# mmbajo/PROBA-V

Hardware: AMD Instinct MI355X
Metric: LR-patches/sec fwd+bwd (WDSR-B r12 t9, 16x16, bs128) (higher is better)
Workload: dtype f32 (products as 3 scaled-fp16-piece MFMA products, f32 accumulate)

## Files before the change

proba-v_amd/csrc/kernels_cw4.hip:

```cpp
#include "kernels_x6.h"
#include "x6_device.h"
#include <cstdlib>
#include <algorithm>

namespace probav {
#ifdef CW4_DIAG
namespace diag {
#endif

struct Cw4Args {
    ConvGeom g;
    int Wp, Wt, nsplit, SR, nstrips, nslot;
    unsigned mTo, mNvr, mTi, mNslot;
};

namespace {
__device__ __forceinline__ int qdiv(int v, int d, unsigned m) { return (int)__umulhi((unsigned)v, m) + (d == 1 ? v : 0); }
unsigned qmagic(int d) { return d <= 1 ? 0u : (unsigned)((0x100000000ull + (unsigned)d - 1) / (unsigned)d); }
typedef float f32x4u __attribute__((ext_vector_type(4), aligned(4)));
typedef unsigned u32x4b __attribute__((ext_vector_type(4)));
constexpr int CW4_PSE = 151;
constexpr int CW4_PS = 16 * CW4_PSE;
constexpr int CW4_ROW = 8 * CW4_PS;
constexpr unsigned CW4_OOB = 0x40000000u;
}

#ifdef CW4_STAMP
__device__ unsigned long long g_cw4_stamps[1024 * 8];
#endif

#define CW4_SBAR() __builtin_amdgcn_sched_barrier(0)
#ifdef CW4_STAMP
#define CW4_ST(k) do { unsigned long long t_; asm volatile("s_memtime %0\n\ts_waitcnt lgkmcnt(0)" : "=s"(t_) :: "memory"); st_acc[k] += t_ - st_prev; st_prev = t_; } while (0)
#ifdef CW4_STAMP_ROUNDS
#define CW4_STR(k) CW4_ST(k)
#else
#define CW4_STR(k) do { } while (0)
#endif
#else
#define CW4_STR(k) do { } while (0)
#define CW4_ST(k) do { } while (0)
#endif

template <int CIN, int COUT, int TP, bool RELU, bool SKIP, bool BIAS>
__global__ __launch_bounds__(256, 1) void conv3_w4_kernel(Cw4Args a, const float* __restrict__ x, const uint4* __restrict__ wfrag, const float* __restrict__ bias,
                                                         const float* __restrict__ skip, float* __restrict__ y, Amax am)
{
    extern __shared__ __attribute__((aligned(16))) unsigned char lds[];
    constexpr int NST = CIN == 25 ? 5 : 6, KB = 9 * NST, G = 3 * KB;
    constexpr int NW1R = CIN == 25 ? 12 : 8;
    constexpr int NCH = CIN == 25 ? 3 : 4;
    constexpr int PS = CW4_PS, ROW = CW4_ROW;
    constexpr int PD = 2;
    constexpr int TO = TP - 2;
    const ConvGeom& g = a.g;
    const int tid = threadIdx.x, lane = tid & 63, half = lane >> 5, col = lane & 31;
    const int wave = __builtin_amdgcn_readfirstlane(tid >> 6);
    const int per = a.nstrips * a.nsplit;
    const int n = blockIdx.x / per, srem = blockIdx.x - n * per;
    const int strip = srem / a.nsplit, sp = srem - strip * a.nsplit;
    const int ws0 = sp * a.Wt, hb = strip * a.SR;
    const int SRr = g.Ho - hb < a.SR ? g.Ho - hb : a.SR;
    const int nvr = a.Wt * g.To, NV = SRr * nvr, NTL = (NV + 31) >> 5, nround = (NTL + 3) >> 2;
    const int NS = a.nslot;
    float omax = 0.f;
#ifdef CW4_STAMP
    unsigned long long st_t0 = __builtin_amdgcn_s_memtime(), st_r0 = __builtin_amdgcn_s_memrealtime();
    unsigned long long st_prev = st_t0, st_acc[8] = {0, 0, 0, 0, 0, 0, 0, 0};
#endif

    const int lw0 = a.nsplit == 1 ? g.pw : 0, Wl = a.nsplit == 1 ? g.Wi : a.Wt + 2;
    const int nvs = Wl * g.Ti, items = nvs * NCH;
    const int ea = h3_exp(am.x[n]);
    const float sa = pow2i(ea);
    int s_srcb[2], s_offb[2];
    float s_sc[2];
    int s3_o[3], s3_offb = 0;
    float s3_sc[3] = {0.f, 0.f, 0.f};
    {
        auto locate = [&](int lv, int& lw, int& t, int& iwc, int& colok) {
            const int lwr = qdiv(lv, g.Ti, a.mTi);
            t = lv - lwr * g.Ti; lw = lw0 + lwr;
            const int iw = ws0 + lw - g.pw;
            colok = (iw >= 0 ? 1 : 0) & (iw < g.Wi ? 1 : 0);
            iwc = iw < 0 ? 0 : (iw < g.Wi ? iw : g.Wi - 1);
        };
#pragma unroll
        for (int k = 0; k < 2; ++k) {
            const int it = tid + 256 * k;
            const int ic = it < items ? it : items - 1;
            const int lv = CIN == 25 ? (int)(((unsigned)ic * 43691u) >> 17) : ic >> 2;
            const int cc = ic - lv * NCH;
            int lw, t, iwc, colok;
            locate(lv, lw, t, iwc, colok);
            s_srcb[k] = ((iwc * g.Ti + t) * CIN + 8 * cc) * 4;
            s_offb[k] = (lw * TO + t) * 16 + cc * PS;
            s_sc[k] = colok ? sa : 0.f;
        }
        if constexpr (CIN == 25) {
            const int lv = tid < nvs ? tid : nvs - 1;
            int lw, t, iwc, colok;
            locate(lv, lw, t, iwc, colok);
            const int base = ((iwc * g.Ti + t) * CIN + 24) * 4;
            s3_offb = (lw * TO + t) * 16 + 3 * PS;
            const int ok3[3] = {colok && t - 1 >= 0, colok, colok && t + 1 < g.Ti};
#pragma unroll
            for (int j = 0; j < 3; ++j) { s3_o[j] = base + (ok3[j] ? (j - 1) * CIN * 4 : 0); s3_sc[j] = ok3[j] ? sa : 0.f; }
        }
    }
    const long xsample = (long)g.Hi * g.Wi * g.Ti * CIN;
    const __amdgpu_buffer_rsrc_t xrs = __builtin_amdgcn_make_buffer_rsrc(const_cast<float*>(x + (long)n * xsample), 0, (unsigned)xsample * 4u, 0x00020000);
    const int xrowb = g.Wi * g.Ti * CIN * 4;
    struct Staged { u32x4b v[2][2]; unsigned g3[3]; };
    auto row_of = [&](int q, int& rowoff, float& rokf) {
        const int ih = hb - g.ph + q;
        const bool rok = ih >= 0 && ih < g.Hi;
        rowoff = (rok ? ih : 0) * xrowb;
        rokf = rok ? 1.f : 0.f;
    };
    auto stage_load_items = [&](int rowoff, Staged& sv) {
#pragma unroll
        for (int k = 0; k < 2; ++k) {
            sv.v[k][0] = __builtin_amdgcn_raw_buffer_load_b128(xrs, s_srcb[k], rowoff, 0);
            sv.v[k][1] = __builtin_amdgcn_raw_buffer_load_b128(xrs, s_srcb[k] + 16, rowoff, 0);
        }
    };
    auto stage_load_g3 = [&](int rowoff, Staged& sv) {
#ifdef CW4_ABL_NOG3
        sv.g3[0] = sv.g3[1] = sv.g3[2] = 0u; return;
#endif
        if constexpr (CIN == 25) {
#pragma unroll
            for (int j = 0; j < 3; ++j) sv.g3[j] = __builtin_amdgcn_raw_buffer_load_b32(xrs, s3_o[j], rowoff, 0);
        }
    };
    auto slot_of = [&](int q) -> int { return (q - qdiv(q, NS, a.mNslot) * NS) * ROW; };
    struct Cut { float sc[2], sg[3]; f32x2 t[4]; unsigned h0[4], h1[4]; float u[3]; };
    constexpr int ROW_MOPS = CIN == 25 ? 52 : 41;
    auto stage_mop = [&](int m, int slot, float rokf, Staged& sv, Cut& c, bool reload, int rel) {
        if (m < 5) {
            if (m < 2) c.sc[m] = s_sc[m] * rokf;
            else if (CIN == 25) c.sg[m - 2] = s3_sc[m - 2] * rokf;
            return;
        }
        m -= 5;
        if (m < 36) {
            const int k = m / 18, i = m % 18;
            if (i < 16) {
                const int p = i >> 2, op = i & 3;
                if (op == 0) {
                    const u32x4b q = sv.v[k][p >> 1];
                    const f32x2 v = {__uint_as_float(q[2 * (p & 1)]), __uint_as_float(q[2 * (p & 1) + 1])};
                    c.t[p] = v * (f32x2){c.sc[k], c.sc[k]};
                    if (p == 3 && reload) {
                        sv.v[k][0] = __builtin_amdgcn_raw_buffer_load_b128(xrs, s_srcb[k], rel, 0);
                        sv.v[k][1] = __builtin_amdgcn_raw_buffer_load_b128(xrs, s_srcb[k] + 16, rel, 0);
                    }
                } else if (op == 1) {
                    c.h0[p] = __builtin_bit_cast(unsigned, __builtin_convertvector(c.t[p], f16x2));
                } else if (op == 2) {
                    asm("v_fma_mixlo_f16 %0, %1, -1.0, %2 op_sel:[0,0,0] op_sel_hi:[1,0,0]" : "=v"(c.h1[p]) : "v"(c.h0[p]), "v"(c.t[p][0]));
                } else {
                    asm("v_fma_mixhi_f16 %0, %1, -1.0, %2 op_sel:[1,0,0] op_sel_hi:[1,0,0]" : "+v"(c.h1[p]) : "v"(c.h0[p]), "v"(c.t[p][1]));
                }
            } else {
#ifdef CW4_ABL_NOWRITE
                asm volatile("" :: "v"(c.h0[0]), "v"(c.h0[1]), "v"(c.h0[2]), "v"(c.h0[3]), "v"(c.h1[0]), "v"(c.h1[1]), "v"(c.h1[2]), "v"(c.h1[3]));
                return;
#endif
                unsigned char* ent = lds + slot + s_offb[k];
                if (i == 16) *reinterpret_cast<uint4*>(ent) = make_uint4(c.h0[0], c.h0[1], c.h0[2], c.h0[3]);
                else *reinterpret_cast<uint4*>(ent + 4 * PS) = make_uint4(c.h1[0], c.h1[1], c.h1[2], c.h1[3]);
            }
            return;
        }
        if constexpr (CIN == 25) {
            m -= 36;
            if (m < 3) { c.u[m] = __uint_as_float(sv.g3[m]) * c.sg[m]; if (m == 2 && reload) stage_load_g3(rel, sv); }
            else if (m == 3) c.h0[0] = __builtin_bit_cast(unsigned, __builtin_convertvector((f32x2){c.u[0], c.u[1]}, f16x2));
            else if (m == 4) c.h0[1] = __builtin_bit_cast(unsigned, __builtin_convertvector((f32x2){c.u[2], 0.f}, f16x2));
            else if (m == 5) asm("v_fma_mixlo_f16 %0, %1, -1.0, %2 op_sel:[0,0,0] op_sel_hi:[1,0,0]" : "=v"(c.h1[0]) : "v"(c.h0[0]), "v"(c.u[0]));
            else if (m == 6) asm("v_fma_mixhi_f16 %0, %1, -1.0, %2 op_sel:[1,0,0] op_sel_hi:[1,0,0]" : "+v"(c.h1[0]) : "v"(c.h0[0]), "v"(c.u[1]));
            else if (m == 7) c.h1[1] = 0u;
            else if (m == 8) asm("v_fma_mixlo_f16 %0, %1, -1.0, %2 op_sel:[0,0,0] op_sel_hi:[1,0,0]" : "+v"(c.h1[1]) : "v"(c.h0[1]), "v"(c.u[2]));
            else if (m == 9) *reinterpret_cast<uint2*>(lds + slot + s3_offb) = make_uint2(c.h0[0], c.h0[1]);
            else *reinterpret_cast<uint2*>(lds + slot + s3_offb + 4 * PS) = make_uint2(c.h1[0], c.h1[1]);
        }
    };
    auto need = [&](int r) -> int {
        const int vlast = (r + 1) * 128 - 1 < NV - 1 ? (r + 1) * 128 - 1 : NV - 1;
        return qdiv(vlast, nvr, a.mNvr) + 2;
    };

    CW4_ST(3);
    int hiq = nround > 0 ? need(0) : -1;
    Staged p0[4];
    int p0_slot[4];
    float p0_rok[4];
#pragma unroll
    for (int q = 0; q < 4; ++q) {
        int rowoff;
        row_of(q <= hiq ? q : 0, rowoff, p0_rok[q]);
        p0_slot[q] = slot_of(q <= hiq ? q : 0);
        stage_load_items(rowoff, p0[q]);
        stage_load_g3(rowoff, p0[q]);
    }
    constexpr int NQ = ((KB - NW1R) * 64 + 255) / 256;
    u32x4b w1q[NQ];
    const u32x4b* wfrag4 = reinterpret_cast<const u32x4b*>(wfrag);
    const int Z0c = a.Wp * (TP - 2);
    constexpr int NF = KB + NW1R, NF4 = (NF + 3) / 4;
    u32x4b xq[NF4];
#pragma unroll
    for (int i = 0; i < NF4; ++i) {
        int f = 4 * i + wave;
        f = f < NF ? f : NF - 1;
        xq[i] = wfrag4[(f < KB ? 2 * f : 2 * (f - KB) + 1) * 64 + lane];
    }
    const int tab = NS * ROW + (KB - NW1R) * 1024;
    const int tc = tid < g.Cout ? tid : 0;
    const unsigned tew = am.w[tc];
    const float tbv = (bias ? bias : reinterpret_cast<const float*>(am.w))[tc];
#pragma unroll
    for (int i = 0; i < NQ; ++i) {
        int e = tid + 256 * i;
        e = e < (KB - NW1R) * 64 ? e : (KB - NW1R) * 64 - 1;
        w1q[i] = wfrag4[(2 * (NW1R + (e >> 6)) + 1) * 64 + (e & 63)];
    }
    CW4_ST(4);
    if (tid < 32) {
        const int e = -(ea + h3_exp_w(tew));
        reinterpret_cast<int*>(lds + tab)[tid] = e;
        reinterpret_cast<float*>(lds + tab + 128)[tid] = (BIAS && bias && tid < g.Cout) ? ldexpf(tbv, -e) : 0.f;
    }
#pragma unroll
    for (int i = 0; i < NF4; ++i) {
        int f = 4 * i + wave;
        f = f < NF ? f : NF - 1;
        *reinterpret_cast<u32x4b*>(lds + f * 1024 + lane * 16) = xq[i];
    }
    asm volatile("s_waitcnt lgkmcnt(0)\n\ts_barrier" ::: "memory");
    f16x8 w0[KB], w1r[NW1R > 0 ? NW1R : 1];
#pragma unroll
    for (int K = 0; K < KB; ++K) { Frag f; f.u = *reinterpret_cast<const uint4*>(lds + K * 1024 + lane * 16); w0[K] = f.h; }
#pragma unroll
    for (int K = 0; K < NW1R; ++K) { Frag f; f.u = *reinterpret_cast<const uint4*>(lds + (KB + K) * 1024 + lane * 16); w1r[K] = f.h; }
#pragma unroll
    for (int K = 0; K < KB; ++K) asm volatile("" : "+a"(w0[K]));
#pragma unroll
    for (int K = 0; K < NW1R; ++K) asm volatile("" : "+a"(w1r[K]));
    asm volatile("s_waitcnt lgkmcnt(0)\n\ts_barrier" ::: "memory");
    if (a.nsplit == 1) {
        uint4* z = reinterpret_cast<uint4*>(lds);
        for (int i = tid; i < NS * ROW / 16; i += 256) z[i] = make_uint4(0u, 0u, 0u, 0u);
    } else {
        const int nzone = CW4_PSE - Z0c, nplanes = NS * 8;
        for (int i = tid; i < nzone * nplanes; i += 256) {
            const int pl = i / nzone, e = i - pl * nzone;
            *reinterpret_cast<uint4*>(lds + pl * PS + (Z0c + e) * 16) = make_uint4(0u, 0u, 0u, 0u);
        }
        if constexpr (CIN == 25) {
            for (int i = tid; i < Z0c * NS * 2; i += 256) {
                const int pl = i / Z0c, e = i - pl * Z0c;
                *reinterpret_cast<uint4*>(lds + (pl >> 1) * ROW + (3 + 4 * (pl & 1)) * PS + e * 16) = make_uint4(0u, 0u, 0u, 0u);
            }
        }
    }
    asm volatile("s_waitcnt lgkmcnt(0)\n\ts_barrier" ::: "memory");
    CW4_ST(5);
#pragma unroll
    for (int q = 0; q < 4; ++q) {
        Cut c;
#pragma unroll
        for (int m = 0; m < ROW_MOPS; ++m) stage_mop(m, p0_slot[q], p0_rok[q], p0[q], c, false, 0);
    }
    CW4_ST(6);
    const int w1a = NS * ROW + lane * 16;
#pragma unroll
    for (int i = 0; i < NQ; ++i) {
        int e = tid + 256 * i;
        e = e < (KB - NW1R) * 64 ? e : (KB - NW1R) * 64 - 1;
        *reinterpret_cast<u32x4b*>(lds + NS * ROW + e * 16) = w1q[i];
    }
    int eun[16];
    f32x16 bias16;
#pragma unroll
    for (int jj = 0; jj < 4; ++jj) {
        const int4 e4 = *reinterpret_cast<const int4*>(lds + tab + (8 * jj + 4 * half) * 4);
        const float4 b4 = *reinterpret_cast<const float4*>(lds + tab + 128 + (8 * jj + 4 * half) * 4);
        eun[4 * jj] = e4.x; eun[4 * jj + 1] = e4.y; eun[4 * jj + 2] = e4.z; eun[4 * jj + 3] = e4.w;
        bias16[4 * jj] = b4.x; bias16[4 * jj + 1] = b4.y; bias16[4 * jj + 2] = b4.z; bias16[4 * jj + 3] = b4.w;
    }
    const float lo = g.relu ? 0.f : -__builtin_inff();
    (void)lo;
    if (BIAS) asm volatile("" : "+a"(bias16));
    CW4_ST(7);
    asm volatile("s_waitcnt lgkmcnt(0)\n\ts_barrier" ::: "memory");

    const long out_base = ((long)n * g.Ho + hb) * g.Wo * g.To;
    const unsigned ybytes = (unsigned)(SRr * g.Wo * g.To * g.Cout) * 4u;
    const __amdgpu_buffer_rsrc_t yrs = __builtin_amdgcn_make_buffer_rsrc(y + out_base * g.Cout, 0, ybytes, 0x00020000);
    const __amdgpu_buffer_rsrc_t srs = __builtin_amdgcn_make_buffer_rsrc(const_cast<float*>(skip ? skip + out_base * g.Cout : y), 0, skip ? ybytes : 0u, 0x00020000);
    unsigned cofs[4];
#pragma unroll
    for (int jj = 0; jj < 4; ++jj) cofs[jj] = 8 * jj + 4 * half < COUT ? 4u * (8 * jj + 4 * half) : CW4_OOB;

    int offH[5];
    {
        const int pA[5] = {0, 2, 1, 0, 2}, pB[5] = {1, 0, 2, 1, 3};
#pragma unroll
        for (int st = 0; st < 5; ++st) offH[st] = (half ? pB[st] : pA[st]) * PS;
    }
    const int Z0 = a.Wp * TO;
    struct TileTmp { int vi, hrel, rem, w, t, x, e0, s0, s1, s2, b0, b1, b2, dlo, dhi; unsigned yo; };
    constexpr int TILE_STEPS = 14;
    auto tile_step = [&](int step, int tile, TileTmp& q, int (&bs)[9], unsigned (&eo)[4]) {
#define CW4_PIN(v) asm volatile("" : "+v"(v))
        if (step == 0) { const int v = tile * 32 + col; q.vi = v < NV ? v : NV - 1; q.yo = v < NV ? 0u : CW4_OOB; CW4_PIN(q.vi); CW4_PIN(q.yo); }
        if (step == 1) { q.hrel = (int)__umulhi((unsigned)q.vi, a.mNvr); q.rem = q.vi - q.hrel * nvr; CW4_PIN(q.hrel); CW4_PIN(q.rem); }
        if (step == 2) { q.w = (int)__umulhi((unsigned)q.rem, a.mTo); q.t = q.rem - q.w * g.To; CW4_PIN(q.w); CW4_PIN(q.t); }
        if (step == 3) { q.x = q.w * TO + q.t; q.s0 = q.hrel - (int)__umulhi((unsigned)q.hrel, a.mNslot) * NS; CW4_PIN(q.x); CW4_PIN(q.s0); }
        if (step == 4) { q.s1 = q.s0 + 1 < NS ? q.s0 + 1 : q.s0 + 1 - NS; q.e0 = q.x * 16 + (CIN == 32 ? half * PS : 0); CW4_PIN(q.s1); CW4_PIN(q.e0); }
        if (step == 5) { q.s2 = q.s1 + 1 < NS ? q.s1 + 1 : q.s1 + 1 - NS; CW4_PIN(q.s2); }
        if (step == 6) { q.b0 = q.s0 * ROW + q.e0; q.b1 = q.s1 * ROW + q.e0; q.b2 = q.s2 * ROW + q.e0; bs[1] = q.b0; bs[4] = q.b1; bs[7] = q.b2; CW4_PIN(bs[1]); CW4_PIN(bs[4]); CW4_PIN(bs[7]); }
        if (step == 7) { const int z = ((q.x - 1 - Z0) & 15) + Z0 - q.x; q.dlo = q.t == 0 ? z * 16 : -16; CW4_PIN(q.dlo); }
        if (step == 8) { const int z = ((q.x + 1 - Z0) & 15) + Z0 - q.x; q.dhi = q.t == TO - 1 ? z * 16 : 16; CW4_PIN(q.dhi); }
        if (step == 9) { bs[0] = q.b0 + q.dlo; bs[3] = q.b1 + q.dlo; bs[6] = q.b2 + q.dlo; CW4_PIN(bs[0]); CW4_PIN(bs[3]); CW4_PIN(bs[6]); }
        if (step == 10) { bs[2] = q.b0 + q.dhi; bs[5] = q.b1 + q.dhi; bs[8] = q.b2 + q.dhi; CW4_PIN(bs[2]); CW4_PIN(bs[5]); CW4_PIN(bs[8]); }
        if (step == 11) { q.yo += (unsigned)(((q.hrel * g.Wo + ws0 + q.w) * g.To + q.t) * COUT) * 4u; CW4_PIN(q.yo); }
        if (step == 12) { eo[0] = q.yo + cofs[0]; eo[1] = q.yo + cofs[1]; CW4_PIN(eo[0]); CW4_PIN(eo[1]); }
        if (step == 13) { eo[2] = q.yo + cofs[2]; eo[3] = q.yo + cofs[3]; CW4_PIN(eo[2]); CW4_PIN(eo[3]); }
#undef CW4_PIN
    };
    int adr5[5] = {0, 0, 0, 0, 0};
    auto read_A = [&](const int (&bs)[9], int K, Frag (&af)[2]) {
        const int gg = K / NST, st = K % NST, dh = gg / 3, dw = gg % 3;
        if constexpr (CIN == 25) {
            if (dw == 0) {
                const int bm = bs[3 * dh], bz = bs[3 * dh + 1], bp = bs[3 * dh + 2];
                const int b = st == 0 ? bm : st == 1 ? (half ? bz : bm) : st == 2 ? bz : st == 3 ? bp : (half ? bz : bp);
                adr5[st] = b + offH[st];
            }
            const unsigned char* p = lds + adr5[st];
            af[0].u = *reinterpret_cast<const uint4*>(p + dw * TO * 16);
            af[1].u = *reinterpret_cast<const uint4*>(p + dw * TO * 16 + 4 * PS);
        } else {
            const int d = st >> 1, kb = st & 1;
            const unsigned char* p = lds + bs[3 * dh + d];
            af[0].u = *reinterpret_cast<const uint4*>(p + dw * TO * 16 + 2 * kb * PS);
            af[1].u = *reinterpret_cast<const uint4*>(p + dw * TO * 16 + 2 * kb * PS + 4 * PS);
        }
    };
    auto read_W1 = [&](int K, Frag& wf) {
        if (K >= NW1R) wf.u = *reinterpret_cast<const uint4*>(lds + w1a + (K - NW1R) * 1024);
    };

    CW4_ST(2);
    f32x16 accA, accB;
#pragma unroll
    for (int i = 0; i < 16; ++i) { accA[i] = 0.f; accB[i] = 0.f; }
#ifdef CW4_ABL_2ACC
    f32x16 acc2;
    for (int i = 0; i < 16; ++i) acc2[i] = 0.f;
#endif
    f32x4u skq[4];
#pragma unroll
    for (int jj = 0; jj < 4; ++jj) skq[jj] = (f32x4u){0.f, 0.f, 0.f, 0.f};
    int bs[9];
    unsigned eo[4], eo_prev[4] = {CW4_OOB, CW4_OOB, CW4_OOB, CW4_OOB};
    {
        TileTmp q;
#pragma unroll
        for (int st = 0; st < TILE_STEPS; ++st) tile_step(st, wave, q, bs, eo);
    }
    Frag A[PD + 1][2], W1[PD + 1];
#pragma unroll
    for (int K = 0; K < PD; ++K) { read_A(bs, K, A[K]); read_W1(K, W1[K]); }

    Staged sv[2];
    auto round = [&](int r, f32x16& acc, f32x16& pacc) __attribute__((always_inline)) {
        const int hi_next = r + 1 < nround ? need(r + 1) : hiq;
        const int hi_nn = r + 2 < nround ? need(r + 2) : hi_next;
        const int q0 = hiq + 1, q1 = hi_next - hiq >= 2 ? hiq + 2 : hiq + 1;
        const int n0 = hi_next + 1, n1 = hi_nn - hi_next >= 2 ? hi_next + 2 : hi_next + 1;
        int rowoff[2], slot[2];
        float rokf[2], rokn;
        int dummy;
        row_of(q0, dummy, rokf[0]); row_of(q1, dummy, rokf[1]);
        row_of(n0, rowoff[0], rokn); row_of(n1, rowoff[1], rokn);
        slot[0] = slot_of(q0); slot[1] = slot_of(q1);
        Cut cut;
        TileTmp tq;
        int nbs[9];
        unsigned neo[4];
        float m2 = 0.f;
#pragma unroll
        for (int K = 0; K < KB; ++K) {
#pragma unroll
            for (int j = 0; j < 3; ++j) {
                const int gp = 3 * K + j;
                const int sl = K % (PD + 1);
                {
                    f16x8 wa;
                    if (j == 1) { if (K < NW1R) wa = w1r[K < NW1R ? K : 0]; else wa = W1[sl].h; }
                    else wa = w0[K];
                    const f16x8 xb = (j == 0) ? A[sl][1].h : A[sl][0].h;
                    if (gp == 0) {
                        if (BIAS) acc = __builtin_amdgcn_mfma_f32_32x32x16_f16(wa, xb, bias16, 0, 0, 0);
                        else {
                            f32x16 zero;
#pragma unroll
                            for (int i = 0; i < 16; ++i) zero[i] = 0.f;
                            acc = __builtin_amdgcn_mfma_f32_32x32x16_f16(wa, xb, zero, 0, 0, 0);
                        }
                    } else acc = __builtin_amdgcn_mfma_f32_32x32x16_f16(wa, xb, acc, 0, 0, 0);
                }
                CW4_SBAR();
#ifndef CW4_ABL_NOREAD
                if (j == 0) {
                    const int KN = K + PD, sn = KN % (PD + 1);
#ifndef CW4_ABL_W1LATE
                    read_W1(KN < KB ? KN : KN - KB, W1[sn]);
#endif
                    if (KN < KB) read_A(bs, KN, A[sn]); else read_A(nbs, KN - KB, A[sn]);
                }
#ifdef CW4_ABL_W1LATE
                if (j == 1) {
                    const int KN = K + PD, sn = KN % (PD + 1);
                    read_W1(KN < KB ? KN : KN - KB, W1[sn]);
                }
#endif
#endif
                if (K >= 1 && K <= 10 && j == 1) tile_step(K - 1, 4 * (r + 1) + wave, tq, nbs, neo);
                if (K >= 12 && K <= 15 && j == 1) tile_step(K - 2, 4 * (r + 1) + wave, tq, nbs, neo);
                if (K == 11 && j == 1) { CW4_STR(3); asm volatile("s_barrier" ::: "memory"); CW4_STR(4); }
#ifndef CW4_ABL_NOEPI
                if (K < 16 && j == 2) {
                    const int e = K, jj = e >> 2, i = e & 3;
                    float v = ldexpf(pacc[e], eun[e]);
                    if (RELU) v = fmaxf(v, lo);
                    const float o = SKIP ? v + skq[jj][i] : v;
                    skq[jj][i] = o;
                    if ((e & 1) == 0) m2 = o; else asm volatile("v_max3_f32 %0, %0, |%1|, |%2|" : "+v"(omax) : "v"(m2), "v"(o));
                }
                if (j == 1 && (K == 4 || K == 8 || K == 12 || K == 16)) {
                    const int jj = K / 4 - 1;
                    const u32x4b o = {__float_as_uint(skq[jj][0]), __float_as_uint(skq[jj][1]), __float_as_uint(skq[jj][2]), __float_as_uint(skq[jj][3])};
                    if (COUT == 32 || jj < 3) __builtin_amdgcn_raw_buffer_store_b128(o, yrs, eo_prev[jj], 0, 0);
                    else __builtin_amdgcn_raw_buffer_store_b32(o[0], yrs, eo_prev[jj], 0, 0);
                    if (K == 16) omax = r == 0 ? 0.f : omax;
                }
                if (SKIP && (K == 17 || K == 18) && j > 0) {
                    const int jj = 2 * (K - 17) + j - 1;
                    if (COUT == 32 || jj < 3) {
                        const u32x4b q = __builtin_amdgcn_raw_buffer_load_b128(srs, eo[jj], 0, 0);
                        skq[jj] = (f32x4u){__uint_as_float(q[0]), __uint_as_float(q[1]), __uint_as_float(q[2]), __uint_as_float(q[3])};
                    } else {
                        const unsigned q = __builtin_amdgcn_raw_buffer_load_b32(srs, eo[jj], 0, 0);
                        skq[jj] = (f32x4u){__uint_as_float(q), 0.f, 0.f, 0.f};
                    }
                }
#endif
#ifndef CW4_ABL_NOSTAGE
                {
                    constexpr int NKS = (2 * ROW_MOPS + 5) / 6, KS0 = KB - PD - NKS;
                    if (K >= KS0 && K < KS0 + NKS && j > 0) {
                        const int m0 = (K - KS0) * 6 + 3 * (j - 1);
#pragma unroll
                        for (int m = m0; m < m0 + 3; ++m)
                            if (m < 2 * ROW_MOPS) {
#ifdef CW4_ABL_NOCUT
                                if (m == 0) asm volatile("" :: "v"(sv[0].v[0][0]), "v"(sv[0].v[1][1]), "v"(sv[1].v[0][0]), "v"(sv[1].v[1][1]));
                                continue;
#endif
                                stage_mop(m % ROW_MOPS, slot[m / ROW_MOPS], rokf[m / ROW_MOPS], sv[m / ROW_MOPS], cut, true, rowoff[m / ROW_MOPS]);
                            }
                    }
                }
#endif
                CW4_SBAR();
            }
        }
        CW4_STR(5);
#pragma unroll
        for (int d = 0; d < 9; ++d) bs[d] = nbs[d];
#pragma unroll
        for (int jj = 0; jj < 4; ++jj) { eo_prev[jj] = eo[jj]; eo[jj] = neo[jj]; }
        hiq = hi_next;
    };
    {
        const int hi1 = 1 < nround ? need(1) : hiq;
        const int n0 = hiq + 1, n1 = hi1 - hiq >= 2 ? hiq + 2 : hiq + 1;
        int ro;
        float rk;
        row_of(n0, ro, rk); stage_load_items(ro, sv[0]); stage_load_g3(ro, sv[0]);
        row_of(n1, ro, rk); stage_load_items(ro, sv[1]); stage_load_g3(ro, sv[1]);
    }
#pragma unroll 1
    for (int r = 0; r < nround; r += 2) {
        round(r, accA, accB);
        round(r + 1, accB, accA);
    }
    {
#pragma unroll
        for (int e = 0; e < 16; ++e) {
            const int jj = e >> 2, i = e & 3;
            float v = ldexpf(accB[e], eun[e]);
            if (RELU) v = fmaxf(v, lo);
            const float o = SKIP ? v + skq[jj][i] : v;
            skq[jj][i] = o;
            omax = fmaxf(omax, fabsf(o));
        }
        if (nround == 0) omax = 0.f;
#pragma unroll
        for (int jj = 0; jj < 4; ++jj) {
            const u32x4b o = {__float_as_uint(skq[jj][0]), __float_as_uint(skq[jj][1]), __float_as_uint(skq[jj][2]), __float_as_uint(skq[jj][3])};
            if (COUT == 32 || jj < 3) __builtin_amdgcn_raw_buffer_store_b128(o, yrs, eo_prev[jj], 0, 0);
            else __builtin_amdgcn_raw_buffer_store_b32(o[0], yrs, eo_prev[jj], 0, 0);
        }
    }
#ifdef CW4_ABL_2ACC
    for (int i = 0; i < 16; ++i) omax += acc2[i];
#endif
    if (am.y) amax_commit(omax, am.y + n);
#ifdef CW4_STAMP
    if (lane == 0 && blockIdx.x < 256) {
        unsigned long long* o = g_cw4_stamps + (blockIdx.x * 4 + wave) * 8;
        o[0] = __builtin_amdgcn_s_memtime() - st_t0; o[1] = __builtin_amdgcn_s_memrealtime() - st_r0;
        for (int k = 2; k < 8; ++k) o[k] = st_acc[k];
    }
#endif
}

static bool cw4_plan(const ConvGeom& g, Cw4Args& p, size_t& lds_bytes, int& grid)
{
    if (g.kh != 3 || g.kw != 3 || g.kt != 3 || g.reflect_hw || g.reflect_t) return false;
    if (!((g.Cin == 25 && g.Cout == 32) || (g.Cin == 32 && (g.Cout == 25 || g.Cout == 32)))) return false;
    if (g.ph != 1 || g.pw != 1 || g.pt != 1) return false;
    if (g.Ho != g.Hi || g.Wo != g.Wi || g.To != g.Ti) return false;
    if (g.To != 9 && g.To != 7) return false;
    if (g.Ho < 3) return false;
    const int Tp = g.To + 2;
    for (int ns = 1; ns <= 4; ++ns) {
        if (g.Wo % ns) continue;
        const int wt = g.Wo / ns, nvr = wt * g.To;
        const int wp = wt + 2;
        const int nvs = (ns == 1 ? g.Wi : wt + 2) * g.Ti, items = nvs * (g.Cin == 25 ? 3 : 4);
        if (items > 512 || nvs > 256 || nvr < 64 || wp * g.To + 16 + 2 * g.To > CW4_PSE) continue;
        int nstrips = (256 + g.N * ns - 1) / (g.N * ns);
        if (nstrips < 1) nstrips = 1;
        if (nstrips > g.Ho / 4) nstrips = g.Ho / 4 > 0 ? g.Ho / 4 : 1;
        const int SR = (g.Ho + nstrips - 1) / nstrips;
        nstrips = (g.Ho + SR - 1) / SR;
        const int NV = SR * nvr, nround = ((NV + 31) / 32 + 3) / 4;
        auto needf = [&](int r) { const int vl = std::min(NV - 1, (r + 1) * 128 - 1); return vl / nvr + 2; };
        int nslot = needf(0) + 1;
        for (int r = 0; r + 1 < nround; ++r) nslot = std::max(nslot, needf(r + 1) - (r * 128) / nvr + 1);
        const int kb = g.Cin == 25 ? 45 : 54, nw1r = g.Cin == 25 ? 12 : 8;
        const size_t need = (size_t)nslot * CW4_ROW + (size_t)(kb - nw1r) * 1024 + 256;
        if (need > 163840) continue;
        p.g = g; p.Wp = wp; p.Wt = wt; p.nsplit = ns; p.SR = SR; p.nstrips = nstrips; p.nslot = nslot;
        p.mTo = qmagic(g.To); p.mNvr = qmagic(nvr); p.mTi = qmagic(g.Ti); p.mNslot = qmagic(nslot);
        lds_bytes = need; grid = g.N * nstrips * ns;
        return true;
    }
    return false;
}

bool cw4_conv_supported(const ConvGeom& g, const float* gate)
{
    Cw4Args p;
    size_t lds_bytes;
    int grid;
    return gate == nullptr && cw4_plan(g, p, lds_bytes, grid);
}

int cw4_conv_forward(const ConvGeom& g, const float* x, const float* wfrag, const float* bias, const float* skip, float* y, const Amax& am, hipStream_t s)
{
    Cw4Args p;
    size_t lds_bytes;
    int grid;
    if (!cw4_plan(g, p, lds_bytes, grid)) { set_error("cw4_conv_forward: unsupported geometry", hipSuccess); return PROBAV_EINVAL; }
    if (!am.x || !am.w) { set_error("cw4_conv_forward: H3 arithmetic needs the operands' amax slots", hipSuccess); return PROBAV_EINVAL; }
#define CW4_LAUNCH(C, O, T, R, S, B) return launch_lds<conv3_w4_kernel<C, O, T, R, S, B>>("conv3_w4", dim3(grid), dim3(256), lds_bytes, s, p, x, (const uint4*)wfrag, bias, skip, y, am)
#define CW4_LAUNCH_T(C, O) do { if (g.To == 9) CW4_LAUNCH(C, O, 11, true, true, true); else CW4_LAUNCH(C, O, 9, true, true, true); } while (0)
    if (g.Cin == 25 && g.To == 9 && !g.relu && skip && bias) CW4_LAUNCH(25, 32, 11, false, true, true);
    else if (g.Cin == 32 && g.Cout == 25 && g.To == 9 && !g.relu && !skip && !bias) CW4_LAUNCH(32, 25, 11, false, false, false);
    else if (g.Cin == 25) CW4_LAUNCH_T(25, 32);
    else if (g.Cout == 25) CW4_LAUNCH_T(32, 25);
    else CW4_LAUNCH_T(32, 32);
#undef CW4_LAUNCH_T
#undef CW4_LAUNCH
}

#ifdef CW4_DIAG
}
#endif
}
```

Measured before the change: 20180.

## Reorder conv prologue to overlap weight loads with LDS clearing and staging

Moves the global weight-fragment loads to the very start of the kernel and splits the LDS ring clear into an early part (regions not used for fragment staging) and a late part. Fragment readback from LDS is interleaved with the w1 global loads. The first four staged rows are kept in registers (CutRow) and written to LDS only after the late clear. The goal is to hide global-load latency and remove a barrier from the kernel prologue. In exchange it raises register pressure and makes the LDS aliasing between fragments and the ring more delicate.

```diff
diff --git a/proba-v_amd/csrc/kernels_cw4.hip b/proba-v_amd/csrc/kernels_cw4.hip
--- a/proba-v_amd/csrc/kernels_cw4.hip
+++ b/proba-v_amd/csrc/kernels_cw4.hip
@@ -69,6 +69,22 @@
     unsigned long long st_prev = st_t0, st_acc[8] = {0, 0, 0, 0, 0, 0, 0, 0};
 #endif
 
+    const u32x4b* wfrag4 = reinterpret_cast<const u32x4b*>(wfrag);
+    constexpr int NF = KB + NW1R, NF4 = (NF + 3) / 4;
+    const int tc = tid < g.Cout ? tid : 0;
+    const unsigned tew = am.w[tc];
+    const float tbv = (bias ? bias : reinterpret_cast<const float*>(am.w))[tc];
+    auto frag_of = [&](int i) -> int {
+        const int f = 4 * i + wave;
+        return f < NF ? f : NF - 1;
+    };
+    u32x4b xq[NF4];
+#pragma unroll
+    for (int i = 0; i < NF4; ++i) {
+        const int f = frag_of(i);
+        xq[i] = wfrag4[(f < KB ? 2 * f : 2 * (f - KB) + 1) * 64 + lane];
+    }
+    CW4_SBAR();
     const int lw0 = a.nsplit == 1 ? g.pw : 0, Wl = a.nsplit == 1 ? g.Wi : a.Wt + 2;
     const int nvs = Wl * g.Ti, items = nvs * NCH;
     const int ea = h3_exp(am.x[n]);
@@ -205,82 +221,115 @@
         stage_load_items(rowoff, p0[q]);
         stage_load_g3(rowoff, p0[q]);
     }
-    constexpr int NQ = ((KB - NW1R) * 64 + 255) / 256;
-    u32x4b w1q[NQ];
-    const u32x4b* wfrag4 = reinterpret_cast<const u32x4b*>(wfrag);
-    const int Z0c = a.Wp * (TP - 2);
-    constexpr int NF = KB + NW1R, NF4 = (NF + 3) / 4;
-    u32x4b xq[NF4];
-#pragma unroll
-    for (int i = 0; i < NF4; ++i) {
-        int f = 4 * i + wave;
-        f = f < NF ? f : NF - 1;
-        xq[i] = wfrag4[(f < KB ? 2 * f : 2 * (f - KB) + 1) * 64 + lane];
-    }
+    CW4_SBAR();
     const int tab = NS * ROW + (KB - NW1R) * 1024;
-    const int tc = tid < g.Cout ? tid : 0;
-    const unsigned tew = am.w[tc];
-    const float tbv = (bias ? bias : reinterpret_cast<const float*>(am.w))[tc];
-#pragma unroll
-    for (int i = 0; i < NQ; ++i) {
-        int e = tid + 256 * i;
-        e = e < (KB - NW1R) * 64 ? e : (KB - NW1R) * 64 - 1;
-        w1q[i] = wfrag4[(2 * (NW1R + (e >> 6)) + 1) * 64 + (e & 63)];
-    }
-    CW4_ST(4);
     if (tid < 32) {
         const int e = -(ea + h3_exp_w(tew));
         reinterpret_cast<int*>(lds + tab)[tid] = e;
         reinterpret_cast<float*>(lds + tab + 128)[tid] = (BIAS && bias && tid < g.Cout) ? ldexpf(tbv, -e) : 0.f;
     }
-#pragma unroll
-    for (int i = 0; i < NF4; ++i) {
-        int f = 4 * i + wave;
-        f = f < NF ? f : NF - 1;
-        *reinterpret_cast<u32x4b*>(lds + f * 1024 + lane * 16) = xq[i];
-    }
+    const int Z0c = a.Wp * (TP - 2);
+    constexpr int XB = NF * 1024;
+    constexpr int XPL = (XB + PS - 1) / PS;
+    constexpr int XGP = 2 * (XB / ROW) + (XB % ROW <= 3 * PS ? 0 : XB % ROW <= 7 * PS ? 1 : 2);
+    auto clear_ring = [&](bool late) {
+        if (a.nsplit == 1) {
+            uint4* z = reinterpret_cast<uint4*>(lds);
+            const int cut = NS * ROW < XB ? NS * ROW / 16 : XB / 16;
+            for (int i = (late ? 0 : cut) + tid; i < (late ? cut : NS * ROW / 16); i += 256) z[i] = make_uint4(0u, 0u, 0u, 0u);
+        } else {
+            const int nzone = CW4_PSE - Z0c, nplanes = NS * 8;
+            const int zcut = nzone * (XPL < nplanes ? XPL : nplanes);
+            for (int i = (late ? 0 : zcut) + tid; i < (late ? zcut : nzone * nplanes); i += 256) {
+                const int pl = i / nzone, e = i - pl * nzone;
+                *reinterpret_cast<uint4*>(lds + pl * PS + (Z0c + e) * 16) = make_uint4(0u, 0u, 0u, 0u);
+            }
+            if constexpr (CIN == 25) {
+                const int gcut = Z0c * (XGP < NS * 2 ? XGP : NS * 2);
+                for (int i = (late ? 0 : gcut) + tid; i < (late ? gcut : Z0c * NS * 2); i += 256) {
+                    const int pl = i / Z0c, e = i - pl * Z0c;
+                    *reinterpret_cast<uint4*>(lds + (pl >> 1) * ROW + (3 + 4 * (pl & 1)) * PS + e * 16) = make_uint4(0u, 0u, 0u, 0u);
+                }
+            }
+        }
+    };
+    clear_ring(false);
+    CW4_SBAR();
+    CW4_ST(4);
+#pragma unroll
+    for (int i = 0; i < NF4; ++i) *reinterpret_cast<u32x4b*>(lds + frag_of(i) * 1024 + lane * 16) = xq[i];
     asm volatile("s_waitcnt lgkmcnt(0)\n\ts_barrier" ::: "memory");
+    constexpr int NQ = ((KB - NW1R) * 64 + 255) / 256, RPQ = (NF + NQ - 1) / NQ;
+    u32x4b w1q[NQ];
     f16x8 w0[KB], w1r[NW1R > 0 ? NW1R : 1];
-#pragma unroll
-    for (int K = 0; K < KB; ++K) { Frag f; f.u = *reinterpret_cast<const uint4*>(lds + K * 1024 + lane * 16); w0[K] = f.h; }
-#pragma unroll
-    for (int K = 0; K < NW1R; ++K) { Frag f; f.u = *reinterpret_cast<const uint4*>(lds + (KB + K) * 1024 + lane * 16); w1r[K] = f.h; }
+    auto w1_elem = [&](int i) -> int {
+        const int e = tid + 256 * i;
+        return e < (KB - NW1R) * 64 ? e : (KB - NW1R) * 64 - 1;
+    };
+#pragma unroll
+    for (int i = 0; i < NQ; ++i) {
+        const int e = w1_elem(i);
+        w1q[i] = wfrag4[(2 * (NW1R + (e >> 6)) + 1) * 64 + (e & 63)];
+#pragma unroll
+        for (int K = i * RPQ; K < (i + 1) * RPQ && K < NF; ++K) {
+            Frag f;
+            f.u = *reinterpret_cast<const uint4*>(lds + K * 1024 + lane * 16);
+            if (K < KB) w0[K] = f.h; else w1r[K - KB] = f.h;
+        }
+        CW4_SBAR();
+    }
 #pragma unroll
     for (int K = 0; K < KB; ++K) asm volatile("" : "+a"(w0[K]));
 #pragma unroll
     for (int K = 0; K < NW1R; ++K) asm volatile("" : "+a"(w1r[K]));
-    asm volatile("s_waitcnt lgkmcnt(0)\n\ts_barrier" ::: "memory");
-    if (a.nsplit == 1) {
-        uint4* z = reinterpret_cast<uint4*>(lds);
-        for (int i = tid; i < NS * ROW / 16; i += 256) z[i] = make_uint4(0u, 0u, 0u, 0u);
-    } else {
-        const int nzone = CW4_PSE - Z0c, nplanes = NS * 8;
-        for (int i = tid; i < nzone * nplanes; i += 256) {
-            const int pl = i / nzone, e = i - pl * nzone;
-            *reinterpret_cast<uint4*>(lds + pl * PS + (Z0c + e) * 16) = make_uint4(0u, 0u, 0u, 0u);
-        }
-        if constexpr (CIN == 25) {
-            for (int i = tid; i < Z0c * NS * 2; i += 256) {
-                const int pl = i / Z0c, e = i - pl * Z0c;
-                *reinterpret_cast<uint4*>(lds + (pl >> 1) * ROW + (3 + 4 * (pl & 1)) * PS + e * 16) = make_uint4(0u, 0u, 0u, 0u);
-            }
-        }
-    }
-    asm volatile("s_waitcnt lgkmcnt(0)\n\ts_barrier" ::: "memory");
     CW4_ST(5);
+    struct CutRow { u32x4b h0[2], h1[2]; unsigned g0[2], g1[2]; };
+    CutRow cr[4];
 #pragma unroll
     for (int q = 0; q < 4; ++q) {
         Cut c;
 #pragma unroll
-        for (int m = 0; m < ROW_MOPS; ++m) stage_mop(m, p0_slot[q], p0_rok[q], p0[q], c, false, 0);
-    }
+        for (int m = 0; m < ROW_MOPS; ++m) {
+            const int mm = m - 5;
+            if (mm >= 0 && mm < 36 && mm % 18 >= 16) {
+                const int k = mm / 18;
+                if (mm % 18 == 16) cr[q].h0[k] = (u32x4b){c.h0[0], c.h0[1], c.h0[2], c.h0[3]};
+                else cr[q].h1[k] = (u32x4b){c.h1[0], c.h1[1], c.h1[2], c.h1[3]};
+            } else if (mm >= 36 + 9) {
+                if (mm == 36 + 9) { cr[q].g0[0] = c.h0[0]; cr[q].g0[1] = c.h0[1]; }
+                else { cr[q].g1[0] = c.h1[0]; cr[q].g1[1] = c.h1[1]; }
+            } else stage_mop(m, 0, p0_rok[q], p0[q], c, false, 0);
+        }
+    }
+#pragma unroll
+    for (int q = 0; q < 4; ++q) {
+        asm volatile("" :: "v"(cr[q].h0[0]), "v"(cr[q].h0[1]), "v"(cr[q].h1[0]), "v"(cr[q].h1[1]));
+        if constexpr (CIN == 25) asm volatile("" :: "v"(cr[q].g0[0]), "v"(cr[q].g0[1]), "v"(cr[q].g1[0]), "v"(cr[q].g1[1]));
+    }
+    CW4_SBAR();
+    asm volatile("s_waitcnt lgkmcnt(0)\n\ts_barrier" ::: "memory");
     CW4_ST(6);
+    clear_ring(true);
+    asm volatile("s_waitcnt lgkmcnt(0)\n\ts_barrier" ::: "memory");
+#ifndef CW4_ABL_NOWRITE
+#pragma unroll
+    for (int q = 0; q < 4; ++q) {
+#pragma unroll
+        for (int k = 0; k < 2; ++k) {
+            unsigned char* ent = lds + p0_slot[q] + s_offb[k];
+            *reinterpret_cast<u32x4b*>(ent) = cr[q].h0[k];
+            *reinterpret_cast<u32x4b*>(ent + 4 * PS) = cr[q].h1[k];
+        }
+        if constexpr (CIN == 25) {
+            *reinterpret_cast<uint2*>(lds + p0_slot[q] + s3_offb) = make_uint2(cr[q].g0[0], cr[q].g0[1]);
+            *reinterpret_cast<uint2*>(lds + p0_slot[q] + s3_offb + 4 * PS) = make_uint2(cr[q].g1[0], cr[q].g1[1]);
+        }
+    }
+#endif
     const int w1a = NS * ROW + lane * 16;
 #pragma unroll
     for (int i = 0; i < NQ; ++i) {
-        int e = tid + 256 * i;
-        e = e < (KB - NW1R) * 64 ? e : (KB - NW1R) * 64 - 1;
-        *reinterpret_cast<u32x4b*>(lds + NS * ROW + e * 16) = w1q[i];
+        *reinterpret_cast<u32x4b*>(lds + NS * ROW + w1_elem(i) * 16) = w1q[i];
     }
     int eun[16];
     f32x16 bias16;
```

Result: no change. 20300, median of 6 (+0.6%).
